# ianic/flate

Measured on AMD Instinct MI355X. Metric: MB/s uncompressed, deflate level 6 compress, higher is better.
Workload: dtype u8; 1 GPU; raw deflate level 6, 1024 MiB synthetic enwik-like text per GPU, 65535-byte independent chunks (16385 chunks), one MI355X per rank (BASELINE.json configs[1]); container=raw, chunk_bytes=65535, bytes_per_gpu=1073741824, gather=none

## Files before the change

### flate_amd/csrc/flate_common.h

```cpp
#pragma once
#include <stdint.h>

#if defined(__HIPCC__)
#define FL_HD __host__ __device__ inline
#else
#define FL_HD inline
#endif

#define FL_TOK_LIT(b) ((uint32_t)(b) << 15)
#define FL_TOK_MATCH(dist, len) ((1u << 23) | ((uint32_t)((len)-3) << 15) | (uint32_t)((dist)-1))
#define FL_TOK_IS_MATCH(t) (((t) >> 23) & 1u)
#define FL_TOK_LENLIT(t) (((t) >> 15) & 0xffu)
#define FL_TOK_DIST0(t) ((t)&0x7fffu)

#if defined(__HIP_DEVICE_COMPILE__)
#define FL_PLAN_PARALLEL 1
#define FL_PLAN_LANE() (__builtin_amdgcn_mbcnt_hi(~0u, __builtin_amdgcn_mbcnt_lo(~0u, 0u)))
#define FL_PLAN_SYNC()                                        \
    do {                                                      \
        __builtin_amdgcn_fence(__ATOMIC_RELEASE, "wavefront"); \
        __builtin_amdgcn_wave_barrier();                      \
        __builtin_amdgcn_fence(__ATOMIC_ACQUIRE, "wavefront"); \
    } while (0)
#define FL_PLAN_FOR(i, a, b) for (uint32_t i = (a) + FL_PLAN_LANE(); i < (b); i += 64)
// ... 14 lines not shown

#if defined(__HIP_DEVICE_COMPILE__) && defined(FL_PLAN_PROF)
extern __device__ uint64_t g_fl_prof[];
#define FL_PLAN_MARK(slot)                                                                          \
    do {                                                                                            \
        if (blockIdx.x == 0 && threadIdx.x == 0) g_fl_prof[slot] = __builtin_readcyclecounter();    \
    } while (0)
#else
#define FL_PLAN_MARK(slot)
#endif
#define FL_MAX_TOKENS 32768u
#define FL_MIN_MATCH 4u
#define FL_MAX_MATCH 258u
#define FL_MAX_DIST 32768u
#define FL_MAX_STORE 65535u
#define FL_NUM_LIT 286
#define FL_NUM_DIST 30
#define FL_NUM_CG 19
#define FL_EOB 256
#define FL_END_MARK 255

enum { FL_BLOCK_STORED = 0, FL_BLOCK_FIXED = 1, FL_BLOCK_DYNAMIC = 2 };

struct fl_hcode {
    uint16_t code;
    uint16_t len;
};

FL_HD uint32_t fl_len_extra_bits(uint32_t idx) {
    return idx < 8 ? 0u : (idx == 28 ? 0u : (idx - 4) >> 2);
}
FL_HD uint32_t fl_len_base_scaled(uint32_t idx) {
    if (idx < 8) return idx;
    if (idx == 28) return 255;
    uint32_t e = (idx - 4) >> 2;
    return ((4 + ((idx - 4) & 3)) << e);
}
FL_HD uint32_t fl_len_index(uint32_t len_lit) {
    if (len_lit < 8) return len_lit;
    if (len_lit == 255) return 28;
    uint32_t hb = 31u - (uint32_t)__builtin_clz(len_lit);
    return ((hb - 1) << 2) + ((len_lit >> (hb - 2)) & 3);
}
FL_HD uint32_t fl_dist_extra_bits(uint32_t code) { return code < 4 ? 0u : (code - 2) >> 1; }
FL_HD uint32_t fl_dist_base_scaled(uint32_t code) {
    if (code < 4) return code;
    uint32_t e = (code - 2) >> 1;
    return (2 + (code & 1)) << e;
}
FL_HD uint32_t fl_dist_code(uint32_t d) {
    if (d < 4) return d;
    uint32_t hb = 31u - (uint32_t)__builtin_clz(d);
    return (hb << 1) + ((d >> (hb - 1)) & 1);
}

FL_HD uint16_t fl_bit_reverse(uint16_t v, uint32_t n) {
    uint32_t x = v;
    x = ((x & 0x5555u) << 1) | ((x >> 1) & 0x5555u);
    x = ((x & 0x3333u) << 2) | ((x >> 2) & 0x3333u);
    x = ((x & 0x0f0fu) << 4) | ((x >> 4) & 0x0f0fu);
    x = ((x & 0x00ffu) << 8) | ((x >> 8) & 0x00ffu);
    return (uint16_t)(x >> (16 - n));
}

FL_HD fl_hcode fl_fixed_lit_code(uint32_t ch) {
    uint32_t bits, size;
    if (ch <= 143) { bits = ch + 48; size = 8; }
    else if (ch <= 255) { bits = ch + 400 - 144; size = 9; }
    else if (ch <= 279) { bits = ch - 256; size = 7; }
    else { bits = ch + 192 - 280; size = 8; }
    fl_hcode c;
    c.code = fl_bit_reverse((uint16_t)bits, size);
    c.len = (uint16_t)size;
    return c;
}
FL_HD fl_hcode fl_fixed_dist_code(uint32_t ch) {
    fl_hcode c;
    c.code = fl_bit_reverse((uint16_t)ch, 5);
    c.len = 5;
    return c;
}

FL_HD uint32_t fl_codegen_order(uint32_t i) {
    const uint8_t order[19] = {16, 17, 18, 0, 8, 7, 9, 6, 10, 5, 11, 4, 12, 3, 13, 2, 14, 1, 15};
    return order[i];
}

struct fl_level_info {
    uint32_t level, last_freq, next_char_freq, next_pair_freq, needed;
};
struct fl_plan_ws {
    uint16_t lit_freq[FL_NUM_LIT];
    uint16_t dist_freq[FL_NUM_DIST];
    uint16_t cg_freq[FL_NUM_CG];
    fl_hcode lit_codes[FL_NUM_LIT];
    fl_hcode dist_codes[FL_NUM_DIST];
    fl_hcode cg_codes[FL_NUM_CG];
    uint8_t codegen[FL_NUM_LIT + FL_NUM_DIST + 2];
    uint16_t list_sym[FL_NUM_LIT + 1];
    uint16_t list_freq[FL_NUM_LIT + 1];
    uint32_t bit_count[17];
#if !FL_PLAN_PARALLEL
    fl_level_info levels[18];
    uint32_t leaf_counts[17][16];
#endif
    uint32_t pm_w[2 * FL_NUM_LIT];
// ... 676 lines not shown
```

### flate_amd/csrc/flate_hip.hip

```cpp
#include <hip/hip_runtime.h>

#include <dlfcn.h>

#include <algorithm>
#include <cstdio>
#include <cstdlib>
#include <cstring>
#include <string>
#include <chrono>
#include <deque>
#include <vector>
#include <thread>
#include <functional>

#include "../../include/flate_hip.h"
#include "kernels_block.h"
#include "kernels_common.h"
#include "kernels_deflater.h"
#include "kernels_inflate.h"
#include "kernels_inflate_par.h"
#include "kernels_inflate_size.h"
#include "kernels_lz.h"
#include "kernels_parse.h"
#include "kernels_walk.h"
#include "kernels_stream.h"
#include "pass_plan.h"
#include "size_plan.h"
#include "stream_tables.h"

namespace {

enum KernelId {
    K_MEMSET = 0,
    K_BYTE_HIST,
    K_CHECKSUM,
    K_LZ_SORT,
    K_LZ_MATCH,
    K_LZ_CHAIN,
    K_LZ_PARSE,
    K_LZ_LINKS,
    K_LZ_WALK,
    K_LZ_EMIT,
    K_ST_PARSE,
    K_ST_EMIT,
    K_PLAN,
    K_OFFSETS,
    K_ENCODE,
    K_INFLATE,
    K_INFLATE_PAR,
    K_SPAN_SCAN,
    K_INFLATE_SPAN,
    K_INFLATE_SIZE,
    K_INFLATE_SIZE_SPAN,
    K_GATHER,
    K_INFLATER,
    K_DEFLATER,
    K_COUNT
};
const char* const kKernelNames[K_COUNT] = {"memset_out", "k_byte_hist", "k_checksum", "k_lz_sort", "k_lz_match",
                                           "k_lz_chain", "k_lz_parse", "k_lz_links", "k_lz_walk", "k_lz_emit",
                                           "k_st_parse", "k_st_emit", "k_plan",
// ... 3240 lines not shown
```

### flate_amd/csrc/kernels_block.h

```cpp
#pragma once
#include "kernels_common.h"

struct fl_sb {
    uint32_t start, len;
    bool final_block, marker;
};
__device__ __forceinline__ fl_sb fl_simple_block(const fl_chunk& ck, const fl_sblock* __restrict__ sblocks, uint32_t b) {
    fl_sb r;
    if (sblocks) {
        const fl_sblock e = sblocks[b];
        r.start = e.start;
        r.len = e.len;
        r.final_block = (e.flags & 1) != 0;
        r.marker = (e.flags & 2) != 0;
    } else {
        const uint32_t j = b - ck.first_block;
        const uint64_t s = (uint64_t)j * FL_BLOCK_BYTES;
        r.start = (uint32_t)min(s, (uint64_t)ck.in_len);
        r.len = min(FL_BLOCK_BYTES, ck.in_len - r.start);
        r.final_block = j + 1 == ck.n_blocks;
        r.marker = false;
    }
    return r;
}
// ... 639 lines not shown
        nb += fl_block_item<TOKENS>(i, n_hdr, hdr_nbits, n_sym, hdr, bytes, toks, lit_lds, dist_lds).n;
    nb = fl_wave_sum(nb);
    if (lane == 0) wave_bits[wave] = nb;
    __syncthreads();
    uint64_t cur = bit_off;
    for (uint32_t w = 0; w < wave; w++) cur += wave_bits[w];
    if (i0 >= i1) return;

    const uint64_t first_dw = cur >> 5;
    uint32_t* sw = stg[wave];
    for (uint32_t ib = i0; ib < i1; ib += 64) {
        const uint32_t i = ib + lane;
        fl_item it;
        it.v = 0;
        it.n = 0;
        if (i < i1) it = fl_block_item<TOKENS>(i, n_hdr, hdr_nbits, n_sym, hdr, bytes, toks, lit_lds, dist_lds);
        const uint32_t incl = fl_wave_incl_scan(it.n, lane);
        const uint32_t total = __shfl(incl, 63, 64);
        const uint64_t base_dw = cur >> 5;
        if (it.n) {
            const uint32_t rel = (uint32_t)(cur - (base_dw << 5)) + (incl - it.n);
            const uint32_t dw = rel >> 5, sh = rel & 31;
            const uint64_t a = it.v << sh;
            const uint32_t hi = sh ? (uint32_t)(it.v >> (64 - sh)) : 0u;
            if ((uint32_t)a) atomicOr(&sw[dw], (uint32_t)a);
            if ((uint32_t)(a >> 32)) atomicOr(&sw[dw + 1], (uint32_t)(a >> 32));
            if (hi) atomicOr(&sw[dw + 2], hi);
        }
        fl_lds_order();
        const uint64_t end = cur + total;
        const uint32_t nd = (uint32_t)((end >> 5) - base_dw);
        for (uint32_t k = lane; k < nd; k += 64) {
            const uint32_t v = sw[k];
            if (base_dw + k == first_dw) {
                if (v) atomicOr(&out32[base_dw + k], v);
            } else {
                out32[base_dw + k] = v;
            }
        }
        const uint32_t carry = sw[nd];
        fl_lds_order();
        for (uint32_t k = lane; k <= nd + 2 && k < FL_STG_DW; k += 64) sw[k] = 0;
        fl_lds_order();
        if (lane == 0) sw[0] = carry;
        fl_lds_order();
        cur = end;
    }
    if ((cur & 31) && lane == 0) {
        const uint32_t v = sw[0];
        if (v) atomicOr(&out32[cur >> 5], v);
    }
}

__global__ __launch_bounds__(64 * FL_ENC_WAVES) void k_encode_wave(const uint8_t* __restrict__ in,
                                                              const fl_chunk* __restrict__ chunks,
                                                              const uint32_t* __restrict__ blk_chunk,
                                                              const fl_block_plan* __restrict__ plans,
                                                              const uint32_t* __restrict__ tokens ,
                                                              uint32_t* __restrict__ out32, uint32_t n_blocks,
                                                              uint32_t pair_slots) {
    __shared__ uint32_t lit_all[FL_ENC_WAVES][FL_NUM_LIT + 2];
    __shared__ uint32_t dist_all[FL_ENC_WAVES][FL_NUM_DIST + 2];
    __shared__ uint32_t stg[FL_ENC_WAVES][FL_STG_DW];

    const uint32_t tid = threadIdx.x, lane = tid & 63, wave = tid >> 6;
    uint32_t b = blockIdx.x * FL_ENC_WAVES + wave;
    if (b >= n_blocks) return;
    if (pair_slots) {
        const uint32_t half = n_blocks >> 1;
        b = b < half ? 2 * b : 2 * (b - half) + 1;
    }
    const fl_block_plan* plan = &plans[b];
    if (!plan->valid) return;
    const uint32_t cidx = blk_chunk[b];
    const fl_chunk ck = chunks[cidx];
    uint32_t* lit_lds = lit_all[wave];
    uint32_t* dist_lds = dist_all[wave];
    const uint64_t bit_off = plan->bit_off;
    const uint8_t* src = in + ck.in_off;

    if (plan->type == FL_BLOCK_STORED) {
        const uint32_t len = plan->in_len;
        const uint64_t p = (bit_off + 3 + 7) >> 3;
        if (lane == 0) {
            if (plan->final_block) fl_atomic_or_bits(out32, bit_off, 1, 1);
            const uint32_t lw = (len & 0xffff) | ((~len & 0xffff) << 16);
            fl_atomic_or_bits(out32, p * 8, lw, 32);
        }
        fl_copy_bytes(out32, p + 4, src + plan->in_start, len, lane, 64);
        return;
    }

    for (uint32_t i = lane; i < FL_NUM_LIT; i += 64)
        lit_lds[i] = (uint32_t)plan->lit[i].code | ((uint32_t)plan->lit[i].len << 16);
    if (lane < FL_NUM_DIST) dist_lds[lane] = (uint32_t)plan->dist[lane].code | ((uint32_t)plan->dist[lane].len << 16);
    for (uint32_t i = lane; i < FL_STG_DW; i += 64) stg[wave][i] = 0;
    fl_lds_order();

    const uint32_t hdr_nbits = plan->hdr_nbits;
    const uint32_t n_hdr = (hdr_nbits + 7) >> 3;
    const uint32_t n_sym = plan->tok_count;
    const uint32_t* toks = tokens + ck.pos_off + plan->tok_start;
    const uint8_t* hdr = plan->hdr;

    uint64_t cur = bit_off;

    const uint64_t first_dw = cur >> 5;
    uint32_t* sw = stg[wave];
    auto pack = [&](const fl_item& it) {
        const uint32_t incl = fl_wave_incl_scan(it.n, lane);
        const uint32_t total = (uint32_t)__builtin_amdgcn_readlane((int)incl, 63);
        const uint64_t base_dw = cur >> 5;
        if (it.n) {
            const uint32_t rel = (uint32_t)(cur - (base_dw << 5)) + (incl - it.n);
            const uint32_t dw = rel >> 5, sh = rel & 31;
            const uint64_t a = it.v << sh;
            const uint32_t hi = sh ? (uint32_t)(it.v >> (64 - sh)) : 0u;
            if ((uint32_t)a) atomicOr(&sw[dw], (uint32_t)a);
            if ((uint32_t)(a >> 32)) atomicOr(&sw[dw + 1], (uint32_t)(a >> 32));
            if (hi) atomicOr(&sw[dw + 2], hi);
        }
        fl_lds_order();
        const uint64_t end = cur + total;
        const uint32_t nd = (uint32_t)((end >> 5) - base_dw);
        {
            const uint32_t v0 = lane < nd ? sw[lane] : 0u, v1 = lane + 64u < nd ? sw[lane + 64u] : 0u;
            if (lane < nd) {
                if (base_dw + lane == first_dw) {
                    if (v0) atomicOr(&out32[base_dw + lane], v0);
                } else {
                    out32[base_dw + lane] = v0;
                }
            }
            if (lane + 64u < nd) out32[base_dw + lane + 64u] = v1;
        }
        const uint32_t carry = sw[nd];
        fl_lds_order();
        if (lane <= nd + 2) sw[lane] = lane == 0 ? carry : 0u;
        if (lane + 64u <= nd + 2 && lane + 64u < FL_STG_DW) sw[lane + 64u] = 0u;
        fl_lds_order();
        cur = end;
    };
    for (uint32_t ib = 0; ib < n_hdr; ib += 64) {
        fl_item it;
        it.v = 0;
        it.n = 0;
        const uint32_t i = ib + lane;
        if (i < n_hdr) {
            const uint32_t rem = hdr_nbits - 8 * i;
            it.n = rem < 8 ? rem : 8;
            it.v = hdr[i] & ((1u << it.n) - 1);
        }
        pack(it);
    }
    const uint32_t eob = lit_lds[FL_EOB];
    uint32_t t_next = lane < n_sym ? toks[lane] : 0u;
    for (uint32_t k0 = 0; k0 < n_sym; k0 += 64) {
        const uint32_t t = t_next;
        t_next = k0 + 64 + lane < n_sym ? toks[k0 + 64 + lane] : 0u;
        fl_item it;
        it.v = 0;
        it.n = 0;
        const uint32_t k = k0 + lane;
        if (k < n_sym) {
            if (!FL_TOK_IS_MATCH(t)) {
                const uint32_t e = lit_lds[FL_TOK_LENLIT(t)];
                it.v = e & 0xffff;
                it.n = e >> 16;
            } else {
                const uint32_t ll = FL_TOK_LENLIT(t);
                const uint32_t li = fl_len_index(ll);
                const uint32_t le = lit_lds[257 + li];
                uint64_t v = le & 0xffff;
                uint32_t n = le >> 16;
                v |= (uint64_t)(ll - fl_len_base_scaled(li)) << n;
                n += fl_len_extra_bits(li);
                const uint32_t d = FL_TOK_DIST0(t);
                const uint32_t dc = fl_dist_code(d);
                const uint32_t de = dist_lds[dc];
                v |= (uint64_t)(de & 0xffff) << n;
                n += de >> 16;
                v |= (uint64_t)(d - fl_dist_base_scaled(dc)) << n;
                n += fl_dist_extra_bits(dc);
                it.v = v;
                it.n = n;
            }
        } else if (k == n_sym) {
            it.v = eob & 0xffff;
            it.n = eob >> 16;
        }
        pack(it);
    }
    if ((n_sym & 63u) == 0) {
        fl_item it;
        it.v = lane == 0 ? (eob & 0xffff) : 0u;
        it.n = lane == 0 ? (eob >> 16) : 0u;
        pack(it);
    }
    if ((cur & 31) && lane == 0) {
        const uint32_t v = sw[0];
        if (v) atomicOr(&out32[cur >> 5], v);
    }
}

__global__ __launch_bounds__(1024) void k_scan_lens(const uint64_t* __restrict__ len, uint32_t n,
                                                    uint64_t* __restrict__ dst_off) {
    __shared__ uint64_t wsum[16];
    __shared__ uint64_t carry;
    const uint32_t tid = threadIdx.x, lane = tid & 63, wave = tid >> 6;
    if (tid == 0) carry = 0;
    __syncthreads();
    for (uint32_t base = 0; base < n; base += 1024) {
        const uint32_t i = base + tid;
        const uint64_t v = i < n ? len[i] : 0;
        uint64_t inc = v;
#pragma unroll
        for (int d = 1; d < 64; d <<= 1) {
            const uint64_t t = __shfl_up(inc, d, 64);
            if (lane >= (uint32_t)d) inc += t;
        }
        if (lane == 63) wsum[wave] = inc;
        __syncthreads();
        uint64_t off = carry;
        for (uint32_t w = 0; w < wave; w++) off += wsum[w];
        if (i < n) dst_off[i] = off + inc - v;
        __syncthreads();
        if (tid == 1023) carry = off + inc;
        __syncthreads();
    }
    if (tid == 0) dst_off[n] = carry;
}

#define FL_GATHER_SLICE 16384u
__device__ __forceinline__ void fl_gather_one(const uint8_t* __restrict__ out, const uint64_t* __restrict__ out_off,
                                              const uint64_t* __restrict__ out_len, uint8_t* __restrict__ dst,
                                              const uint64_t* __restrict__ dst_off, uint32_t c, uint32_t by, uint32_t ny,
                                              uint64_t skip = 0) {
    const uint32_t tid = threadIdx.x;
    const uint64_t n0 = out_len[c];
    if (n0 <= skip) return;
    const uint64_t n = n0 - skip;
    const uint8_t* s = out + out_off[c] + skip;
    uint8_t* d = dst + dst_off[c] + skip;
    const uint64_t head = min(n, (uint64_t)((16 - ((uintptr_t)d & 15)) & 15));
    const uint64_t nq = (n - head) >> 4;
    const uint64_t tail0 = head + 16 * nq;
    if (by == 0) {
        if (tid < head) d[tid] = s[tid];
        if (tid < 16 && tail0 + tid < n) d[tail0 + tid] = s[tail0 + tid];
    }
// ... 39 lines not shown
```

### flate_amd/csrc/kernels_common.h

```cpp
#pragma once
#include <hip/hip_runtime.h>
#include <stdint.h>


#include "flate_layout.h"

#define FL_WAVE 64
#define FL_PROF_SLOTS 160
__device__ uint64_t g_fl_prof[FL_PROF_SLOTS];
__device__ __forceinline__ void fl_prof_mark(uint32_t slot) {
    if (blockIdx.x == 0 && threadIdx.x == 0) g_fl_prof[slot] = __builtin_readcyclecounter();
}

__device__ __forceinline__ uint32_t fl_lane() {
    return __builtin_amdgcn_mbcnt_hi(~0u, __builtin_amdgcn_mbcnt_lo(~0u, 0u));
}
__device__ __forceinline__ uint32_t fl_wave_xor(uint32_t v) {
#pragma unroll
    for (int d = 32; d > 0; d >>= 1) v ^= __shfl_xor(v, d, 64);
    return v;
}
__device__ __forceinline__ uint32_t fl_wave_max(uint32_t v) {
#pragma unroll
    for (int d = 32; d > 0; d >>= 1) {
        uint32_t o = __shfl_xor(v, d, 64);
        v = o > v ? o : v;
    }
    return v;
}
__device__ __forceinline__ uint32_t fl_wave_incl_scan_dpp(uint32_t v) {
    v += (uint32_t)__builtin_amdgcn_update_dpp(0, (int)v, 0x111, 0xf, 0xf, false);
    v += (uint32_t)__builtin_amdgcn_update_dpp(0, (int)v, 0x112, 0xf, 0xf, false);
    v += (uint32_t)__builtin_amdgcn_update_dpp(0, (int)v, 0x114, 0xf, 0xf, false);
    v += (uint32_t)__builtin_amdgcn_update_dpp(0, (int)v, 0x118, 0xf, 0xf, false);
    v += (uint32_t)__builtin_amdgcn_update_dpp(0, (int)v, 0x142, 0xa, 0xf, false);
    v += (uint32_t)__builtin_amdgcn_update_dpp(0, (int)v, 0x143, 0xc, 0xf, false);
    return v;
}
__device__ __forceinline__ uint32_t fl_wave_incl_scan(uint32_t v, uint32_t lane) {
    (void)lane;
    return fl_wave_incl_scan_dpp(v);
}
__device__ __forceinline__ uint32_t fl_wave_sum(uint32_t v) {
    return (uint32_t)__builtin_amdgcn_readlane((int)fl_wave_incl_scan_dpp(v), 63);
}
__device__ __forceinline__ void fl_wave_lds_sync() {
    __builtin_amdgcn_fence(__ATOMIC_RELEASE, "workgroup");
    __builtin_amdgcn_wave_barrier();
    __builtin_amdgcn_fence(__ATOMIC_ACQUIRE, "workgroup");
}

__device__ __forceinline__ void fl_lds_order() {
    asm volatile("" ::: "memory");
    __builtin_amdgcn_wave_barrier();
}

__device__ __forceinline__ uint32_t fl_load_u32_unaligned(const uint8_t* p) {
    const uint32_t sh = (uint32_t)((uintptr_t)p & 3);
    const uint32_t* w = (const uint32_t*)(p - sh);
    const uint32_t lo = w[0];
    if (sh == 0) return lo;
    const uint32_t hi = w[1];
    return __builtin_amdgcn_alignbyte(hi, lo, sh);
}

#define FL_CRC_POLY 0xEDB88320u
__device__ __host__ inline uint32_t fl_crc_mulmod(uint32_t a, uint32_t b) {
    uint32_t p = 0;
    for (int i = 0; i < 32; i++) {
        if (a & 0x80000000u) p ^= b;
        a <<= 1;
        b = (b & 1) ? ((b >> 1) ^ FL_CRC_POLY) : (b >> 1);
    }
    return p;
}
__device__ __host__ inline uint32_t fl_crc_xpow8n(const uint32_t* xpow8, uint64_t n) {
    uint32_t p = 0x80000000u;
    for (int j = 0; n; j++, n >>= 1)
        if (n & 1) p = fl_crc_mulmod(xpow8[j & 31], p);
    return p;
}

__device__ __forceinline__ void fl_atomic_or_bits(uint32_t* out32, uint64_t bitpos, uint64_t v, uint32_t nbits) {
    if (nbits == 0) return;
    const uint64_t dw = bitpos >> 5;
    const uint32_t sh = (uint32_t)(bitpos & 31);
    const uint64_t a = v << sh;
    const uint32_t b = sh ? (uint32_t)(v >> (64 - sh)) : 0u;
    if ((uint32_t)a) atomicOr(&out32[dw], (uint32_t)a);
    if ((uint32_t)(a >> 32)) atomicOr(&out32[dw + 1], (uint32_t)(a >> 32));
    if (b) atomicOr(&out32[dw + 2], b);
}

__device__ inline void fl_copy_bytes(uint32_t* out32, uint64_t dst_byte, const uint8_t* src, uint32_t n,
                                     uint32_t tid, uint32_t nthreads) {
    if (n == 0) return;
    const uint64_t dw0 = dst_byte >> 2;
    const uint64_t dw1 = (dst_byte + n + 3) >> 2;
    for (uint64_t dw = dw0 + tid; dw < dw1; dw += nthreads) {
        const int64_t first = (int64_t)(dw << 2) - (int64_t)dst_byte;
        uint32_t v = 0;
        bool full = true;
#pragma unroll
        for (int k = 0; k < 4; k++) {
            const int64_t si = first + k;
            if (si >= 0 && si < (int64_t)n)
                v |= (uint32_t)src[si] << (8 * k);
// ... 10 lines not shown
```

### flate_amd/csrc/kernels_lz.h

```cpp
#pragma once
#include "kernels_common.h"

__device__ __forceinline__ uint32_t fl_hash_le(uint32_t le_word) {
    return (__builtin_bswap32(le_word) * 0x9E3779B1u) >> 17;
}

template <int NB>
__device__ __forceinline__ uint64_t fl_match_any(uint32_t d, uint64_t valid) {
    uint64_t peers = valid;
#pragma unroll
    for (int bit = 0; bit < NB; bit++) {
        const bool s = (d >> bit) & 1;
        const uint64_t m = __ballot(s);
        peers &= s ? m : ~m;
    }
    return peers;
}

__device__ __forceinline__ void fl_wave_excl_scan_lds(uint32_t* cnt, uint32_t n, uint32_t lane) {
    const uint32_t per = (n + 63) / 64;
    uint32_t v[4];
    uint32_t s = 0;
    for (uint32_t k = 0; k < per; k++) {
        const uint32_t i = lane * per + k;
// ... 720 lines not shown
        if (active) {
            const uint32_t rf = (key >> 16) ? ((key & 0xffff0000u) | (0xfffeu - (key & 0xffffu))) : 0u;
            const uint32_t rq = (qkey >> 16) ? ((qkey & 0xffff0000u) | (0xfffeu - (qkey & 0xffffu))) : 0u;
            rec2[p] = make_uint2(rf, rq);
        }
    }
    fl_prof_mark(11);
}

#define FL_PARSE_THREADS 1024

__device__ __forceinline__ uint32_t fl_desc_next(uint32_t d, uint32_t p) {
    if (!d) return p + 1;
    return p + ((d >> 23) & 0xff) + ((d >> 15) & 0xff) + 3;
}

__device__ __forceinline__ uint32_t fl_anchor_desc(const uint2* __restrict__ rec2, uint32_t p, uint2 ra, uint2 rb,
                                                   uint32_t good, uint32_t lazy) {
    const uint32_t r = ra.x;
    if (!r) return 0;
    uint32_t len = r >> 16, dist0 = r & 0x7fff, j = 0, q = p;
    while (len < lazy) {
        const uint32_t sel = len >= good ? 1u : 0u;
        uint32_t r2;
        if (j == 0) {
            r2 = sel ? rb.y : rb.x;
        } else {
            const uint2 rr = rec2[q + 1];
            r2 = sel ? rr.y : rr.x;
        }
        const uint32_t l2 = r2 >> 16;
        if (l2 <= len) break;
        len = l2;
        dist0 = r2 & 0x7fff;
        j++;
        q++;
    }
    return 0x80000000u | (j << 23) | ((len - 3) << 15) | dist0;
}

#define FL_EMIT_WAVES 16
#define FL_EMIT_THREADS (64 * FL_EMIT_WAVES)

__device__ __forceinline__ uint32_t fl_win_byte(const uint32_t* win32, uint32_t off) {
    return (win32[off >> 2] >> (8 * (off & 3))) & 0xff;
}

#ifndef FL_TOK_PART
#define FL_TOK_PART 8192u
#endif
#define FL_TOK_SPAN (FL_TOK_PART / 16u)
#define FL_TOK_R (FL_TOK_SPAN / 64u)
#define FL_TOK_LOOK 256u
#define FL_TOK_WIN_DW ((FL_TOK_PART + FL_TOK_LOOK) / 4u + 2u)
```

### flate_amd/csrc/kernels_parse.h

```cpp
#pragma once
#include "kernels_common.h"
#include "kernels_lz.h"

#define FL_CHAIN_STG_DW 264

typedef __attribute__((address_space(3))) uint32_t fl_lds_u32;
__device__ __forceinline__ uint32_t fl_lds_mskor_rtn(uint32_t* lds_word, uint32_t mask, uint32_t value) {
    uint32_t old;
    fl_lds_u32* a = (fl_lds_u32*)lds_word;
    asm volatile("ds_mskor_rtn_b32 %0, %1, %2, %3" : "=v"(old) : "v"(a), "v"(mask), "v"(value) : "memory");
    return old;
}

#ifndef FL_BULK_MIN_CHAIN
#define FL_BULK_MIN_CHAIN 1024u
#endif

#ifndef FL_CHAIN_WAVES
#define FL_CHAIN_WAVES 8
#endif
#ifndef FL_CHAIN_TB
#define FL_CHAIN_TB 1
#endif
template <bool FLUSH = false>
// ... 1284 lines not shown
    if (STREAM) {
        __syncthreads();
        carry = sh_exit - FL_MAX_DIST;
        if (wi + 1 == sw.nwin && tid == 0) {
            __hip_atomic_store(&gexit[blockIdx.x], sh_exit + FL_MAX_DIST * ws, __ATOMIC_RELAXED, __HIP_MEMORY_SCOPE_AGENT);
            if (fix) atomicAdd(dirty, 1u);
        }
    }
#ifdef PZ_PROF
#pragma unroll
    for (int k = 0; k < 30; k++) {
        const uint32_t v = fl_wave_sum(c_ev[k]);
        if ((tid & 63) == 0) atomicAdd((unsigned long long*)&g_fl_prof[k], (unsigned long long)v);
    }
    if ((tid & 63) == 0) {
        atomicAdd((unsigned long long*)&g_fl_prof[40], (unsigned long long)c_fast);
        atomicAdd((unsigned long long*)&g_fl_prof[41], (unsigned long long)c_walk);
        atomicAdd((unsigned long long*)&g_fl_prof[42], (unsigned long long)c_slow);
        atomicAdd((unsigned long long*)&g_fl_prof[43], (unsigned long long)c_measl);
        atomicAdd((unsigned long long*)&g_fl_prof[44], (unsigned long long)c_loops);
        atomicAdd((unsigned long long*)&g_fl_prof[45], (unsigned long long)c_rounds);
        atomicAdd((unsigned long long*)&g_fl_prof[46], (unsigned long long)c_tspec);
        atomicAdd((unsigned long long*)&g_fl_prof[47], (unsigned long long)c_tstitch);
        atomicAdd((unsigned long long*)&g_fl_prof[48], (unsigned long long)(__builtin_readcyclecounter() - c_t0));
        atomicAdd((unsigned long long*)&g_fl_prof[49], 1ull);
        atomicAdd((unsigned long long*)&g_fl_prof[50], (unsigned long long)c_tfast);
        atomicAdd((unsigned long long*)&g_fl_prof[51], (unsigned long long)c_tmeas);
        atomicAdd((unsigned long long*)&g_fl_prof[52], (unsigned long long)c_ttrans);
        atomicAdd((unsigned long long*)&g_fl_prof[53], (unsigned long long)c_meas);
        atomicAdd((unsigned long long*)&g_fl_prof[54], (unsigned long long)c_trans);
        atomicAdd((unsigned long long*)&g_fl_prof[55], (unsigned long long)c_tstage);
        atomicAdd((unsigned long long*)&g_fl_prof[56], (unsigned long long)c_tjump);
        atomicAdd((unsigned long long*)&g_fl_prof[58], (unsigned long long)c_tb_le2);
        atomicAdd((unsigned long long*)&g_fl_prof[59], (unsigned long long)c_tb_le8);
        atomicAdd((unsigned long long*)&g_fl_prof[60], (unsigned long long)c_tb_le24);
        atomicAdd((unsigned long long*)&g_fl_prof[61], (unsigned long long)c_tb_more);
        atomicAdd((unsigned long long*)&g_fl_prof[62], (unsigned long long)c_nb_le2);
    }
    (void)c_meas; (void)c_trans; (void)c_transl;
#endif
    }
}

#define FL_EMITZ_THREADS 1024

__global__ __launch_bounds__(FL_EMITZ_THREADS, 8) void k_lz_emit(const uint8_t* __restrict__ in,
                                                                 const fl_chunk* __restrict__ chunks, fl_params prm,
                                                                 const uint32_t* __restrict__ desc_all,
                                                                 const uint32_t* __restrict__ true_all,
                                                                 uint32_t* __restrict__ tokens_all,
                                                                 uint32_t* __restrict__ hist_all,
                                                                 fl_block_plan* __restrict__ plans,
                                                                 uint32_t* __restrict__ ntok_all) {
    __shared__ uint32_t winp[FL_TOK_WIN_DW];
    __shared__ uint32_t hist[2][320];
    __shared__ uint32_t wtot[16];
    __shared__ uint16_t alist[16][FL_TOK_SPAN];
    __shared__ uint32_t v1_sh, e1_sh;
    const uint32_t c = blockIdx.x;
    const fl_chunk ck = chunks[c];
    const uint32_t tid = threadIdx.x, lane = tid & 63, wave = tid >> 6;
    fl_block_plan* plan0 = &plans[ck.first_block];
    fl_block_plan* plan1 = &plans[ck.first_block + 1];
    if (ck.skip) {
        if (tid == 0) {
            plan0->valid = 0;
            plan1->valid = 0;
            ntok_all[c] = 0;
        }
        return;
    }
    const uint32_t N = ck.in_len;
    const uint8_t* src = in + ck.in_off;
    const uint32_t* descg = desc_all + ck.pos_off;
    const uint32_t* trueg = true_all + (ck.pos_off >> 5);
    uint32_t* tokens = tokens_all + ck.pos_off;

    for (uint32_t i = tid; i < 640; i += FL_EMITZ_THREADS) (&hist[0][0])[i] = 0;
    if (tid == 0) v1_sh = e1_sh = N;
    uint32_t run0 = 0;
    uint32_t tw_next = 0;
    if (lane < FL_TOK_SPAN / 32u && wave * FL_TOK_SPAN + 32 * lane < min((uint32_t)FL_TOK_PART, N)) tw_next = trueg[((wave * FL_TOK_SPAN) >> 5) + lane];
    for (uint32_t h0 = 0; h0 < N; h0 += FL_TOK_PART) {
        const uint32_t span0 = h0 + wave * FL_TOK_SPAN;
        const uint32_t tw = tw_next;
        {
            const uint32_t h0n = h0 + FL_TOK_PART, h1n = min(h0n + FL_TOK_PART, N), s0n = h0n + wave * FL_TOK_SPAN;
            tw_next = 0;
            if (h0n < N && lane < FL_TOK_SPAN / 32u && s0n + 32 * lane < h1n) tw_next = trueg[(s0n >> 5) + lane];
        }
        uint32_t na = 0;
#pragma unroll
        for (int r = 0; r < (int)FL_TOK_R; r++) {
            const uint32_t wlo = (uint32_t)__builtin_amdgcn_readlane((int)tw, 2 * r);
            const uint32_t whi = (uint32_t)__builtin_amdgcn_readlane((int)tw, 2 * r + 1);
            const uint64_t m64 = (uint64_t)wlo | ((uint64_t)whi << 32);
            const uint32_t below = __builtin_amdgcn_mbcnt_hi(whi, __builtin_amdgcn_mbcnt_lo(wlo, 0u));
            if (__builtin_amdgcn_inverse_ballot_w64(m64)) alist[wave][na + below] = (uint16_t)(r * 64 + lane);
            na += (uint32_t)__popcll(m64);
        }
        fl_lds_order();
        uint32_t d[FL_TOK_R];
#pragma unroll
        for (int k = 0; k < (int)FL_TOK_R; k++) {
            const uint32_t j = 64 * k + lane;
            d[k] = j < na ? descg[span0 + alist[wave][j]] : 0u;
        }
        {
            const uint32_t nb = min(N - h0, FL_TOK_PART + FL_TOK_LOOK);
            constexpr uint32_t WR = (FL_TOK_WIN_DW + FL_EMITZ_THREADS - 1) / FL_EMITZ_THREADS;
            uint32_t wv[WR];
#pragma unroll
            for (uint32_t u = 0; u < WR; u++) {
                const uint32_t i = u * FL_EMITZ_THREADS + tid;
                wv[u] = 4 * i < nb ? fl_load_u32_clamped(src + h0, 4 * i, nb) : 0u;
            }
#pragma unroll
            for (uint32_t u = 0; u < WR; u++) {
                const uint32_t i = u * FL_EMITZ_THREADS + tid;
                if (i < FL_TOK_WIN_DW) winp[i] = wv[u];
            }
        }
        uint32_t cnt = 0;
#pragma unroll
        for (int r = 0; r < (int)FL_TOK_R; r++) cnt += d[r] ? ((d[r] & PZ_DESC_LIT) ? 1u : ((d[r] >> 23) & 0xff) + 1u) : 0u;
        cnt = fl_wave_sum(cnt);
        if (lane == 0) wtot[wave] = cnt;
        __syncthreads();
        uint32_t run = run0;
        for (uint32_t w = 0; w < 16; w++) {
            if (w < wave) run += wtot[w];
            run0 += wtot[w];
        }
#pragma unroll 1
        for (uint32_t k0 = 0; k0 < na; k0 += 64) {
            const uint32_t j = k0 + lane;
            const uint32_t d0r = d[0];
#pragma unroll
            for (int k = 0; k + 1 < (int)FL_TOK_R; k++) d[k] = d[k + 1];
            d[FL_TOK_R - 1] = d0r;
            const bool mk = d0r != 0;
            const uint32_t p = span0 + (mk ? (uint32_t)alist[wave][j] : 0u);
            const uint32_t q = p - h0;
            const uint32_t dd = (d0r & PZ_DESC_LIT) ? 0u : d0r;
            const uint32_t nl = mk ? (dd ? ((dd >> 23) & 0xff) : 1u) : 0u;
            const uint32_t nt = mk ? (dd ? nl + 1 : 1u) : 0u;
            const uint32_t incl = fl_wave_incl_scan_dpp(nt);
            uint32_t idx = run + incl - nt;
            run += __builtin_amdgcn_readlane(incl, 63);
            for (uint32_t x = 0; x < nl; x++) {
                const uint32_t byte = fl_win_byte(winp, q + x);
                tokens[idx] = FL_TOK_LIT(byte);
                atomicAdd(&hist[idx >> 15][byte], 1u);
                if (idx == FL_MAX_TOKENS - 1) v1_sh = e1_sh = p + x + 1;
                idx++;
            }
            if (mk && dd) {
                const uint32_t ll = (dd >> 15) & 0xff, d0 = dd & 0x7fff;
                tokens[idx] = (1u << 23) | (ll << 15) | d0;
                atomicAdd(&hist[idx >> 15][257 + fl_len_index(ll)], 1u);
                atomicAdd(&hist[idx >> 15][286 + fl_dist_code(d0)], 1u);
                if (idx == FL_MAX_TOKENS - 1) {
                    v1_sh = p + nl + ((ll + 3 >= prm.lazy) ? 0 : 1);
                    e1_sh = p + nl + ll + 3;
                }
            }
        }
        __syncthreads();
    }
    const uint32_t total = run0;
    const uint32_t nblk = total >= FL_MAX_TOKENS ? 2 : 1;
    uint32_t* hg = hist_all + (uint64_t)ck.first_block * 320;
    for (uint32_t i = tid; i < 640; i += FL_EMITZ_THREADS)
        if (i < 320 * nblk) hg[i] = (&hist[0][0])[i];
    if (tid == 0) {
        ntok_all[c] = total;
        const bool repair = (prm.flags & FL_PRM_REPAIR_Q1) != 0;
        const uint32_t v1 = repair ? e1_sh : v1_sh;
        plan0->no_input = 0;
        plan1->no_input = 0;
        plan0->q1_gap = (nblk == 2 && !repair) ? e1_sh - v1_sh : 0u;
        plan1->q1_gap = 0;
        if (nblk == 1) {
            plan0->valid = 1;
            plan0->tok_start = 0;
            plan0->tok_count = total;
            plan0->in_start = 0;
            plan0->in_len = N;
            plan0->final_block = 1;
            plan1->valid = 0;
        } else {
            plan0->valid = 1;
            plan0->tok_start = 0;
            plan0->tok_count = FL_MAX_TOKENS;
            plan0->in_start = 0;
            plan0->in_len = v1;
            plan0->final_block = 0;
            plan1->valid = 1;
            plan1->tok_start = FL_MAX_TOKENS;
            plan1->tok_count = total - FL_MAX_TOKENS;
            plan1->in_start = v1;
            plan1->in_len = N - v1;
            plan1->final_block = 1;
        }
    }
}
```

Measured before the change: 42550 MB/s.

## Restructure encode and token-emit kernels with fused code tables and paired tokens

The wave encoder now builds a combined literal/length table with extra bits prebaked, plus a distance table whose code index comes from a float-exponent trick. Each lane processes two tokens per pack step, so scans and barriers run half as often, and the staging buffer grows to 200 dwords. The token-emit kernel loads its input window with 16-byte vector loads and looks up length codes in an LDS table. It also specialises the histogram path for rounds that do not cross the block split, takes a fast path when every lane emits a single literal, and unrolls the rounds. These changes add register and LDS pressure and add code-path complexity around the block-cut logic.

Result: faster. 43870 MB/s, median of 6 (+3.1%).

```diff
diff --git a/flate_amd/csrc/flate_common.h b/flate_amd/csrc/flate_common.h
--- a/flate_amd/csrc/flate_common.h
+++ b/flate_amd/csrc/flate_common.h
@@ -90,6 +90,14 @@
     if (d < 4) return d;
     uint32_t hb = 31u - (uint32_t)__builtin_clz(d);
     return (hb << 1) + ((d >> (hb - 1)) & 1);
+}
+
+FL_HD uint32_t fl_dist_code_p256(uint32_t d) {
+    const float x = (float)((d << 1) | 1u);
+    uint32_t f;
+    __builtin_memcpy(&f, &x, 4);
+    f >>= 22;
+    return f < 256u ? 256u : f;
 }
 
 FL_HD uint16_t fl_bit_reverse(uint16_t v, uint32_t n) {
diff --git a/flate_amd/csrc/flate_hip.hip b/flate_amd/csrc/flate_hip.hip
--- a/flate_amd/csrc/flate_hip.hip
+++ b/flate_amd/csrc/flate_hip.hip
@@ -7,6 +7,7 @@
 #include <cstdlib>
 #include <cstring>
 #include <string>
+#include <type_traits>
 #include <chrono>
 #include <deque>
 #include <vector>
diff --git a/flate_amd/csrc/kernels_block.h b/flate_amd/csrc/kernels_block.h
--- a/flate_amd/csrc/kernels_block.h
+++ b/flate_amd/csrc/kernels_block.h
@@ -715,6 +715,11 @@
     }
 }
 
+#define FL_ENCW_GROUP 128u
+struct __attribute__((packed, aligned(4))) fl_tok2 {
+    uint32_t a, b;
+};
+#define FL_ENCW_STG_DW 200
 __global__ __launch_bounds__(64 * FL_ENC_WAVES) void k_encode_wave(const uint8_t* __restrict__ in,
                                                               const fl_chunk* __restrict__ chunks,
                                                               const uint32_t* __restrict__ blk_chunk,
@@ -722,11 +727,12 @@
                                                               const uint32_t* __restrict__ tokens ,
                                                               uint32_t* __restrict__ out32, uint32_t n_blocks,
                                                               uint32_t pair_slots) {
-    __shared__ uint32_t lit_all[FL_ENC_WAVES][FL_NUM_LIT + 2];
-    __shared__ uint32_t dist_all[FL_ENC_WAVES][FL_NUM_DIST + 2];
-    __shared__ uint32_t stg[FL_ENC_WAVES][FL_STG_DW];
-
-    const uint32_t tid = threadIdx.x, lane = tid & 63, wave = tid >> 6;
+    __shared__ uint32_t tab_all[FL_ENC_WAVES][512];
+    __shared__ uint2 dtab_all[FL_ENC_WAVES][32];
+    __shared__ uint32_t stg[FL_ENC_WAVES][FL_ENCW_STG_DW];
+
+    const uint32_t tid = threadIdx.x, lane = tid & 63;
+    const uint32_t wave = (uint32_t)__builtin_amdgcn_readfirstlane((int)(tid >> 6));
     uint32_t b = blockIdx.x * FL_ENC_WAVES + wave;
     if (b >= n_blocks) return;
     if (pair_slots) {
@@ -737,8 +743,8 @@
     if (!plan->valid) return;
     const uint32_t cidx = blk_chunk[b];
     const fl_chunk ck = chunks[cidx];
-    uint32_t* lit_lds = lit_all[wave];
-    uint32_t* dist_lds = dist_all[wave];
+    uint32_t* tab = tab_all[wave];
+    uint2* dtab = dtab_all[wave];
     const uint64_t bit_off = plan->bit_off;
     const uint8_t* src = in + ck.in_off;
 
@@ -754,10 +760,19 @@
         return;
     }
 
-    for (uint32_t i = lane; i < FL_NUM_LIT; i += 64)
-        lit_lds[i] = (uint32_t)plan->lit[i].code | ((uint32_t)plan->lit[i].len << 16);
-    if (lane < FL_NUM_DIST) dist_lds[lane] = (uint32_t)plan->dist[lane].code | ((uint32_t)plan->dist[lane].len << 16);
-    for (uint32_t i = lane; i < FL_STG_DW; i += 64) stg[wave][i] = 0;
+#pragma unroll
+    for (uint32_t u = 0; u < 4; u++) {
+        const uint32_t i = 64 * u + lane;
+        const fl_hcode lc = plan->lit[i];
+        tab[i] = (uint32_t)lc.code | ((uint32_t)lc.len << 24);
+        const uint32_t li = fl_len_index(i);
+        const fl_hcode mc = plan->lit[257 + li];
+        tab[256 + i] = ((uint32_t)mc.code | ((i - fl_len_base_scaled(li)) << mc.len)) | (((uint32_t)mc.len + fl_len_extra_bits(li)) << 24);
+    }
+    if (lane < FL_NUM_DIST)
+        dtab[lane] = make_uint2((uint32_t)plan->dist[lane].code | ((uint32_t)plan->dist[lane].len << 16),
+                                fl_dist_base_scaled(lane) | (fl_dist_extra_bits(lane) << 16));
+    for (uint32_t i = lane; i < FL_ENCW_STG_DW; i += 64) stg[wave][i] = 0;
     fl_lds_order();
 
     const uint32_t hdr_nbits = plan->hdr_nbits;
@@ -770,95 +785,119 @@
 
     const uint64_t first_dw = cur >> 5;
     uint32_t* sw = stg[wave];
-    auto pack = [&](const fl_item& it) {
-        const uint32_t incl = fl_wave_incl_scan(it.n, lane);
-        const uint32_t total = (uint32_t)__builtin_amdgcn_readlane((int)incl, 63);
-        const uint64_t base_dw = cur >> 5;
-        if (it.n) {
-            const uint32_t rel = (uint32_t)(cur - (base_dw << 5)) + (incl - it.n);
+    auto or_item = [&](const uint32_t rel, const uint64_t v, const uint32_t n) {
+        if (n) {
             const uint32_t dw = rel >> 5, sh = rel & 31;
-            const uint64_t a = it.v << sh;
-            const uint32_t hi = sh ? (uint32_t)(it.v >> (64 - sh)) : 0u;
+            const uint64_t a = v << sh;
+            const uint32_t hi = (uint32_t)(((uint64_t)(uint32_t)(v >> 32) << sh) >> 32);
             if ((uint32_t)a) atomicOr(&sw[dw], (uint32_t)a);
             if ((uint32_t)(a >> 32)) atomicOr(&sw[dw + 1], (uint32_t)(a >> 32));
             if (hi) atomicOr(&sw[dw + 2], hi);
         }
+    };
+    auto pack = [&](const uint64_t va, const uint32_t na, const uint64_t vb, const uint32_t nb) {
+        const uint32_t nn = na + nb;
+        const uint32_t incl = fl_wave_incl_scan(nn, lane);
+        const uint32_t total = (uint32_t)__builtin_amdgcn_readlane((int)incl, 63);
+        const uint64_t base_dw = cur >> 5;
+        const uint32_t rel = ((uint32_t)cur & 31u) + (incl - nn);
+        or_item(rel, va, na);
+        or_item(rel + na, vb, nb);
         fl_lds_order();
         const uint64_t end = cur + total;
         const uint32_t nd = (uint32_t)((end >> 5) - base_dw);
+        uint32_t* o = out32 + base_dw;
         {
-            const uint32_t v0 = lane < nd ? sw[lane] : 0u, v1 = lane + 64u < nd ? sw[lane + 64u] : 0u;
-            if (lane < nd) {
-                if (base_dw + lane == first_dw) {
-                    if (v0) atomicOr(&out32[base_dw + lane], v0);
-                } else {
-                    out32[base_dw + lane] = v0;
+            const uint32_t v0 = lane < nd ? sw[lane] : 0u;
+            if (base_dw == first_dw) {
+                if (lane == 0) {
+                    if (nd && v0) atomicOr(&o[0], v0);
+                } else if (lane < nd) {
+                    fl_st32_off(o, 4u * lane, v0);
                 }
-            }
-            if (lane + 64u < nd) out32[base_dw + lane + 64u] = v1;
+            } else if (lane < nd) {
+                fl_st32_off(o, 4u * lane, v0);
+            }
+            if (nd > 64u) {
+                const uint32_t v1 = lane + 64u < nd ? sw[lane + 64u] : 0u, v2 = lane + 128u < nd ? sw[lane + 128u] : 0u;
+                if (lane + 64u < nd) fl_st32_off(o, 4u * (lane + 64u), v1);
+                if (lane + 128u < nd) fl_st32_off(o, 4u * (lane + 128u), v2);
+            }
         }
         const uint32_t carry = sw[nd];
         fl_lds_order();
         if (lane <= nd + 2) sw[lane] = lane == 0 ? carry : 0u;
-        if (lane + 64u <= nd + 2 && lane + 64u < FL_STG_DW) sw[lane + 64u] = 0u;
+        if (nd + 2 >= 64u) {
+            if (lane + 64u <= nd + 2) sw[lane + 64u] = 0u;
+            if (lane + 128u <= nd + 2 && lane + 128u < FL_ENCW_STG_DW) sw[lane + 128u] = 0u;
+        }
         fl_lds_order();
         cur = end;
     };
     for (uint32_t ib = 0; ib < n_hdr; ib += 64) {
-        fl_item it;
-        it.v = 0;
-        it.n = 0;
+        uint32_t v = 0, n = 0;
         const uint32_t i = ib + lane;
         if (i < n_hdr) {
             const uint32_t rem = hdr_nbits - 8 * i;
-            it.n = rem < 8 ? rem : 8;
-            it.v = hdr[i] & ((1u << it.n) - 1);
-        }
-        pack(it);
-    }
-    const uint32_t eob = lit_lds[FL_EOB];
-    uint32_t t_next = lane < n_sym ? toks[lane] : 0u;
-    for (uint32_t k0 = 0; k0 < n_sym; k0 += 64) {
-        const uint32_t t = t_next;
-        t_next = k0 + 64 + lane < n_sym ? toks[k0 + 64 + lane] : 0u;
-        fl_item it;
-        it.v = 0;
-        it.n = 0;
-        const uint32_t k = k0 + lane;
+            n = rem < 8 ? rem : 8;
+            v = hdr[i] & ((1u << n) - 1);
+        }
+        pack(v, n, 0, 0);
+    }
+    const fl_hcode eobc = plan->lit[FL_EOB];
+    auto token_bits = [&](const uint32_t t, uint64_t& v, uint32_t& n) {
+        const uint32_t e = tab[(t >> 15) & 0x1ffu];
+        v = e & 0xffffffu;
+        n = e >> 24;
+        if (FL_TOK_IS_MATCH(t)) {
+            const uint32_t d = FL_TOK_DIST0(t);
+            const uint2 de = dtab[fl_dist_code_p256(d) - 256u];
+            const uint32_t dl = de.x >> 16;
+            const uint32_t dv = (de.x & 0xffffu) | ((d - (de.y & 0xffffu)) << dl);
+            v |= (uint64_t)dv << n;
+            n += dl + (de.y >> 16);
+        }
+    };
+    auto slot_bits = [&](const uint32_t t, const uint32_t k, uint64_t& v, uint32_t& n) {
+        v = 0;
+        n = 0;
         if (k < n_sym) {
-            if (!FL_TOK_IS_MATCH(t)) {
-                const uint32_t e = lit_lds[FL_TOK_LENLIT(t)];
-                it.v = e & 0xffff;
-                it.n = e >> 16;
-            } else {
-                const uint32_t ll = FL_TOK_LENLIT(t);
-                const uint32_t li = fl_len_index(ll);
-                const uint32_t le = lit_lds[257 + li];
-                uint64_t v = le & 0xffff;
-                uint32_t n = le >> 16;
-                v |= (uint64_t)(ll - fl_len_base_scaled(li)) << n;
-                n += fl_len_extra_bits(li);
-                const uint32_t d = FL_TOK_DIST0(t);
-                const uint32_t dc = fl_dist_code(d);
-                const uint32_t de = dist_lds[dc];
-                v |= (uint64_t)(de & 0xffff) << n;
-                n += de >> 16;
-                v |= (uint64_t)(d - fl_dist_base_scaled(dc)) << n;
-                n += fl_dist_extra_bits(dc);
-                it.v = v;
-                it.n = n;
-            }
+            token_bits(t, v, n);
         } else if (k == n_sym) {
-            it.v = eob & 0xffff;
-            it.n = eob >> 16;
-        }
-        pack(it);
-    }
-    if ((n_sym & 63u) == 0) {
-        fl_item it;
-        it.v = lane == 0 ? (eob & 0xffff) : 0u;
-        it.n = lane == 0 ? (eob >> 16) : 0u;
-        pack(it);
+            v = eobc.code;
+            n = eobc.len;
+        }
+    };
+    auto load2 = [&](const uint32_t k) {
+        fl_tok2 r;
+        r.a = r.b = 0;
+        if (k + 1 < n_sym)
+            r = *(const fl_tok2*)((const char*)toks + 4u * k);
+        else if (k < n_sym)
+            r.a = *(const uint32_t*)((const char*)toks + 4u * k);
+        return r;
+    };
+    fl_tok2 t_next = load2(2 * lane);
+    uint32_t k0 = 0;
+    for (; k0 + FL_ENCW_GROUP <= n_sym; k0 += FL_ENCW_GROUP) {
+        const fl_tok2 t = t_next;
+        t_next = load2(k0 + FL_ENCW_GROUP + 2 * lane);
+        uint64_t va, vb;
+        uint32_t na, nb;
+        token_bits(t.a, va, na);
+        token_bits(t.b, vb, nb);
+        pack(va, na, vb, nb);
+    }
+    if (k0 < n_sym) {
+        const uint32_t k = k0 + 2 * lane;
+        uint64_t va, vb;
+        uint32_t na, nb;
+        slot_bits(t_next.a, k, va, na);
+        slot_bits(t_next.b, k + 1, vb, nb);
+        pack(va, na, vb, nb);
+    }
+    if ((n_sym & (FL_ENCW_GROUP - 1u)) == 0) {
+        pack(lane == 0 ? (uint64_t)eobc.code : 0u, lane == 0 ? (uint32_t)eobc.len : 0u, 0, 0);
     }
     if ((cur & 31) && lane == 0) {
         const uint32_t v = sw[0];
diff --git a/flate_amd/csrc/kernels_common.h b/flate_amd/csrc/kernels_common.h
--- a/flate_amd/csrc/kernels_common.h
+++ b/flate_amd/csrc/kernels_common.h
@@ -53,6 +53,13 @@
 __device__ __forceinline__ void fl_lds_order() {
     asm volatile("" ::: "memory");
     __builtin_amdgcn_wave_barrier();
+}
+
+__device__ __forceinline__ uint32_t fl_ld32_off(const uint32_t* __restrict__ base, uint32_t byte_off) {
+    return *(const uint32_t*)((const char*)base + byte_off);
+}
+__device__ __forceinline__ void fl_st32_off(uint32_t* __restrict__ base, uint32_t byte_off, uint32_t v) {
+    *(uint32_t*)((char*)base + byte_off) = v;
 }
 
 __device__ __forceinline__ uint32_t fl_load_u32_unaligned(const uint8_t* p) {
diff --git a/flate_amd/csrc/kernels_lz.h b/flate_amd/csrc/kernels_lz.h
--- a/flate_amd/csrc/kernels_lz.h
+++ b/flate_amd/csrc/kernels_lz.h
@@ -796,4 +796,3 @@
 #define FL_TOK_SPAN (FL_TOK_PART / 16u)
 #define FL_TOK_R (FL_TOK_SPAN / 64u)
 #define FL_TOK_LOOK 256u
-#define FL_TOK_WIN_DW ((FL_TOK_PART + FL_TOK_LOOK) / 4u + 2u)
diff --git a/flate_amd/csrc/kernels_parse.h b/flate_amd/csrc/kernels_parse.h
--- a/flate_amd/csrc/kernels_parse.h
+++ b/flate_amd/csrc/kernels_parse.h
@@ -1360,14 +1360,18 @@
                                                                  uint32_t* __restrict__ hist_all,
                                                                  fl_block_plan* __restrict__ plans,
                                                                  uint32_t* __restrict__ ntok_all) {
-    __shared__ uint32_t winp[FL_TOK_WIN_DW];
+    constexpr uint32_t WIN_GRAN = (FL_TOK_PART + FL_TOK_LOOK + 15u + 15u) / 16u;
+    static_assert(WIN_GRAN <= FL_EMITZ_THREADS, "one granule a thread");
+    __shared__ uint4 win16[WIN_GRAN];
     __shared__ uint32_t hist[2][320];
     __shared__ uint32_t wtot[16];
     __shared__ uint16_t alist[16][FL_TOK_SPAN];
     __shared__ uint32_t v1_sh, e1_sh;
+    __shared__ uint8_t lent[256];
     const uint32_t c = blockIdx.x;
     const fl_chunk ck = chunks[c];
-    const uint32_t tid = threadIdx.x, lane = tid & 63, wave = tid >> 6;
+    const uint32_t tid = threadIdx.x, lane = tid & 63;
+    const uint32_t wave = (uint32_t)__builtin_amdgcn_readfirstlane((int)(tid >> 6));
     fl_block_plan* plan0 = &plans[ck.first_block];
     fl_block_plan* plan1 = &plans[ck.first_block + 1];
     if (ck.skip) {
@@ -1383,8 +1387,11 @@
     const uint32_t* descg = desc_all + ck.pos_off;
     const uint32_t* trueg = true_all + (ck.pos_off >> 5);
     uint32_t* tokens = tokens_all + ck.pos_off;
+    const uint8_t* winb = (const uint8_t*)win16;
+    uint16_t* al = alist[wave];
 
     for (uint32_t i = tid; i < 640; i += FL_EMITZ_THREADS) (&hist[0][0])[i] = 0;
+    if (tid < 256) lent[tid] = (uint8_t)fl_len_index(tid);
     if (tid == 0) v1_sh = e1_sh = N;
     uint32_t run0 = 0;
     uint32_t tw_next = 0;
@@ -1404,34 +1411,28 @@
             const uint32_t whi = (uint32_t)__builtin_amdgcn_readlane((int)tw, 2 * r + 1);
             const uint64_t m64 = (uint64_t)wlo | ((uint64_t)whi << 32);
             const uint32_t below = __builtin_amdgcn_mbcnt_hi(whi, __builtin_amdgcn_mbcnt_lo(wlo, 0u));
-            if (__builtin_amdgcn_inverse_ballot_w64(m64)) alist[wave][na + below] = (uint16_t)(r * 64 + lane);
+            if (__builtin_amdgcn_inverse_ballot_w64(m64)) al[na + below] = (uint16_t)(r * 64 + lane);
             na += (uint32_t)__popcll(m64);
         }
         fl_lds_order();
+        const uint32_t wsh = (uint32_t)((uintptr_t)(src + h0) & 15u);
+        const uint32_t ngran = (min(N - h0, FL_TOK_PART + FL_TOK_LOOK) + wsh + 15u) >> 4;
+        uint4 wg = make_uint4(0, 0, 0, 0);
+        if (tid < ngran) wg = *(const uint4*)(src + h0 - wsh + (tid << 4));
+        const uint32_t* dspan = descg + span0;
         uint32_t d[FL_TOK_R];
 #pragma unroll
         for (int k = 0; k < (int)FL_TOK_R; k++) {
             const uint32_t j = 64 * k + lane;
-            d[k] = j < na ? descg[span0 + alist[wave][j]] : 0u;
-        }
-        {
-            const uint32_t nb = min(N - h0, FL_TOK_PART + FL_TOK_LOOK);
-            constexpr uint32_t WR = (FL_TOK_WIN_DW + FL_EMITZ_THREADS - 1) / FL_EMITZ_THREADS;
-            uint32_t wv[WR];
-#pragma unroll
-            for (uint32_t u = 0; u < WR; u++) {
-                const uint32_t i = u * FL_EMITZ_THREADS + tid;
-                wv[u] = 4 * i < nb ? fl_load_u32_clamped(src + h0, 4 * i, nb) : 0u;
-            }
-#pragma unroll
-            for (uint32_t u = 0; u < WR; u++) {
-                const uint32_t i = u * FL_EMITZ_THREADS + tid;
-                if (i < FL_TOK_WIN_DW) winp[i] = wv[u];
-            }
-        }
+            d[k] = j < na ? fl_ld32_off(dspan, 4u * al[j]) : 0u;
+        }
+        if (tid < ngran) win16[tid] = wg;
         uint32_t cnt = 0;
 #pragma unroll
-        for (int r = 0; r < (int)FL_TOK_R; r++) cnt += d[r] ? ((d[r] & PZ_DESC_LIT) ? 1u : ((d[r] >> 23) & 0xff) + 1u) : 0u;
+        for (int r = 0; r < (int)FL_TOK_R; r++) {
+            const uint32_t dm = (d[r] & PZ_DESC_LIT) ? 0u : d[r];
+            cnt += (d[r] != 0 ? 1u : 0u) + ((dm >> 23) & 0xffu);
+        }
         cnt = fl_wave_sum(cnt);
         if (lane == 0) wtot[wave] = cnt;
         __syncthreads();
@@ -1440,39 +1441,58 @@
             if (w < wave) run += wtot[w];
             run0 += wtot[w];
         }
-#pragma unroll 1
-        for (uint32_t k0 = 0; k0 < na; k0 += 64) {
-            const uint32_t j = k0 + lane;
-            const uint32_t d0r = d[0];
-#pragma unroll
-            for (int k = 0; k + 1 < (int)FL_TOK_R; k++) d[k] = d[k + 1];
-            d[FL_TOK_R - 1] = d0r;
-            const bool mk = d0r != 0;
-            const uint32_t p = span0 + (mk ? (uint32_t)alist[wave][j] : 0u);
-            const uint32_t q = p - h0;
-            const uint32_t dd = (d0r & PZ_DESC_LIT) ? 0u : d0r;
-            const uint32_t nl = mk ? (dd ? ((dd >> 23) & 0xff) : 1u) : 0u;
-            const uint32_t nt = mk ? (dd ? nl + 1 : 1u) : 0u;
-            const uint32_t incl = fl_wave_incl_scan_dpp(nt);
-            uint32_t idx = run + incl - nt;
-            run += __builtin_amdgcn_readlane(incl, 63);
-            for (uint32_t x = 0; x < nl; x++) {
-                const uint32_t byte = fl_win_byte(winp, q + x);
-                tokens[idx] = FL_TOK_LIT(byte);
-                atomicAdd(&hist[idx >> 15][byte], 1u);
-                if (idx == FL_MAX_TOKENS - 1) v1_sh = e1_sh = p + x + 1;
-                idx++;
-            }
-            if (mk && dd) {
-                const uint32_t ll = (dd >> 15) & 0xff, d0 = dd & 0x7fff;
-                tokens[idx] = (1u << 23) | (ll << 15) | d0;
-                atomicAdd(&hist[idx >> 15][257 + fl_len_index(ll)], 1u);
-                atomicAdd(&hist[idx >> 15][286 + fl_dist_code(d0)], 1u);
-                if (idx == FL_MAX_TOKENS - 1) {
-                    v1_sh = p + nl + ((ll + 3 >= prm.lazy) ? 0 : 1);
-                    e1_sh = p + nl + ll + 3;
-                }
-            }
+        run = (uint32_t)__builtin_amdgcn_readfirstlane((int)run);
+        auto emit_round = [&](const uint32_t dk, const uint32_t k0) {
+            const bool mk = dk != 0;
+            const uint32_t p = span0 + (mk ? (uint32_t)al[k0 + lane] : 0u);
+            const uint32_t q = p - h0 + wsh;
+            const bool one = (dk & PZ_DESC_LIT) != 0;
+            const uint32_t dd = one ? 0u : dk;
+            const uint32_t jl = (dd >> 23) & 0xffu;
+            const uint32_t nl = one ? 1u : jl;
+            const uint32_t nt = (mk ? 1u : 0u) + jl;
+            uint32_t incl = fl_wave_incl_scan_dpp(nt);
+            asm("" : "+v"(incl));
+            const uint32_t idx0 = run + incl - nt;
+            const uint32_t run1 = run + (uint32_t)__builtin_amdgcn_readlane((int)incl, 63);
+            auto body = [&](auto cut_t) {
+                constexpr bool CUT = decltype(cut_t)::value;
+                uint32_t idx = idx0;
+                uint32_t* hs = hist[CUT ? 0u : (run >> 15)];
+                auto literal = [&](const uint32_t x) {
+                    const uint32_t byte = winb[q + x];
+                    fl_st32_off(tokens, 4u * idx, FL_TOK_LIT(byte));
+                    atomicAdd(CUT ? &hist[idx >> 15][byte] : &hs[byte], 1u);
+                    if (CUT && idx == FL_MAX_TOKENS - 1) v1_sh = e1_sh = p + x + 1;
+                    idx++;
+                };
+                if (__builtin_amdgcn_ballot_w64(nl > 1u) == 0) {
+                    if (nl) literal(0u);
+                } else {
+                    for (uint32_t x = 0; x < nl; x++) literal(x);
+                }
+                if (dd) {
+                    const uint32_t ll = (dd >> 15) & 0xff, d0 = dd & 0x7fff;
+                    fl_st32_off(tokens, 4u * idx, (1u << 23) | (dd & 0x7fffffu));
+                    uint32_t* hm = CUT ? hist[idx >> 15] : hs;
+                    atomicAdd(&hm[257 + lent[ll]], 1u);
+                    atomicAdd(&hm[286 - 256 + fl_dist_code_p256(d0)], 1u);
+                    if (CUT && idx == FL_MAX_TOKENS - 1) {
+                        v1_sh = p + nl + ((ll + 3 >= prm.lazy) ? 0 : 1);
+                        e1_sh = p + nl + ll + 3;
+                    }
+                }
+            };
+            if (run < FL_MAX_TOKENS && run1 >= FL_MAX_TOKENS)
+                body(std::true_type());
+            else
+                body(std::false_type());
+            run = run1;
+        };
+#pragma unroll
+        for (int k = 0; k < (int)FL_TOK_R; k++) {
+            if (64u * k >= na) break;
+            emit_round(d[k], 64u * k);
         }
         __syncthreads();
     }
```
